# Audio-WestlakeU/FN-SSL

Measured on AMD Instinct MI355X. Metric: TF-frames/sec DP-IPD forward, 4-mic 257-bin x 300-frame, higher is better.
Workload: dtype f32; 1 GPU; BASELINE configs[1]: FN-SSL (online) DP-IPD forward, waveform->STFT->features->3x(full-band BiLSTM + narrow-band LSTM)->head; 32 utterances/GPU x 4 mics ('MM' = 6 pairs) x 257 bins x 300 frames, fp32; frame = one STFT frame of one utterance; stream_chunk_frames=0, utterances_per_gpu=32, global_batch=32, mics=4, pairs_per_utterance=6, frames=300, bins=257, parallelism=dp1 (utterance shards, no collective), chunk_pairs=0

## Files before the change

fn-ssl_amd/csrc/forward.hip:

```cpp
#include <algorithm>

#include "common.h"

namespace {

size_t align_up(size_t v, size_t a) { return (v + a - 1) / a * a; }

struct Plan {
  int chunk;
  size_t act_floats;
  size_t lstm_ws;
  size_t head_floats;
  size_t total;
};

Plan make_plan(int nb, int nf, int nt, int is_online, int chunk_pairs) {
  Plan p;
  p.chunk = (chunk_pairs <= 0 || chunk_pairs > nb) ? nb : chunk_pairs;
  p.act_floats = (size_t)p.chunk * nt * nf * 256;
  const size_t ws_full = fnssl_lstm_workspace_bytes_ex(p.chunk * nt, 128, 2, FNSSL_PRECISION_FP32);
  const size_t ws_narr = is_online ? fnssl_lstm_workspace_bytes_ex(p.chunk * nf, 256, 1, FNSSL_PRECISION_FP32)
                                   : fnssl_lstm_workspace_bytes_ex(p.chunk * nf, 128, 2, FNSSL_PRECISION_FP32);
  p.lstm_ws = align_up(std::max(ws_full, ws_narr), 256);
  p.head_floats = (size_t)p.chunk * (nt / FNSSL_SEG_FRAMES) * 2 * nf;
  p.total = 6 * align_up(p.act_floats * 4, 256) + p.lstm_ws + align_up(p.head_floats * 4, 256) + 256;
  return p;
}

}

extern "C" {

size_t fnssl_forward_workspace_bytes(int nb, int nf, int nt, int is_online, int chunk_pairs) {
  if (nb <= 0 || nf <= 0 || nt <= 0) return 0;
  return make_plan(nb, nf, nt, is_online, chunk_pairs).total;
}

int fnssl_forward(const fnssl_net* net, const float* x0, int nb, int nf, int nt, float* out, void* workspace,
                  size_t workspace_bytes, int chunk_pairs, void* stream) {
  FNSSL_REQUIRE(net && x0, "forward: null pointer");
  FNSSL_REQUIRE(nb > 0 && nf > 0 && nt > 0, "forward: empty problem (nb %d, nf %d, nt %d)", nb, nf, nt);
  if (nt / FNSSL_SEG_FRAMES == 0) return FNSSL_OK;
  FNSSL_REQUIRE(out, "forward: null output pointer");
  FNSSL_REQUIRE(net->input_size > 0 && net->input_size % 4 == 0, "forward: input_size %d must be a multiple of 4",
                net->input_size);
  FNSSL_REQUIRE(!net->doa_wt || nf == 256, "forward: the DOA layer needs nf = 256 (Linear(512, 180))");
  const Plan pl = make_plan(nb, nf, nt, net->is_online, chunk_pairs);
  if (!workspace || workspace_bytes < pl.total) {
    fnssl::set_error("forward: workspace %zu < %zu bytes", workspace_bytes, pl.total);
    return FNSSL_E_WORKSPACE;
  }
  char* wsb = static_cast<char*>(workspace);
  wsb = reinterpret_cast<char*>(align_up(reinterpret_cast<uintptr_t>(wsb), 256));
  const size_t act_bytes = align_up(pl.act_floats * 4, 256);
  float* F[2] = {reinterpret_cast<float*>(wsb), reinterpret_cast<float*>(wsb + act_bytes)};
  float* N[2] = {reinterpret_cast<float*>(wsb + 2 * act_bytes), reinterpret_cast<float*>(wsb + 3 * act_bytes)};
  float* Sf = reinterpret_cast<float*>(wsb + 4 * act_bytes);
  float* Sn = reinterpret_cast<float*>(wsb + 5 * act_bytes);
  float* lws = reinterpret_cast<float*>(wsb + 6 * act_bytes);
  float* head_tmp = reinterpret_cast<float*>(wsb + 6 * act_bytes + pl.lstm_ws);

  const int cin = net->input_size;
  const int nt2 = nt / FNSSL_SEG_FRAMES;
  const int narr_h = net->is_online ? 256 : 128;
  const int narr_dirs = net->is_online ? 1 : 2;
  const long long C = 256;
  const long long PS = (long long)nt * nf * C;
  const fnssl_view fl_by_full = {nullptr, PS, (long long)nf * C, C};
  const fnssl_view fl_by_narr = {nullptr, PS, C, (long long)nf * C};
  const fnssl_view nl_by_full = {nullptr, PS, C, (long long)nt * C};
  const fnssl_view nl_by_narr = {nullptr, PS, (long long)nt * C, C};
  auto with = [](fnssl_view v, const float* p) {
    v.p = p;
    return v;
  };

  for (int p0 = 0; p0 < nb; p0 += pl.chunk) {
    const int G = std::min(pl.chunk, nb - p0);
    const float* xc = x0 + (size_t)p0 * nt * nf * cin;
    for (int blk = 0; blk < 3; ++blk) {
      float* Fo = F[blk & 1];
      float* No = N[blk & 1];
      const float* Np = N[(blk + 1) & 1];
      fnssl_lstm_desc d = {};
      d.hidden = 128;
      d.ndir = 2;
      d.nseq = G * nt;
      d.q_inner = nt;
      d.nsteps = nf;
      if (blk == 0) {
        d.src0 = fnssl_view{xc, (long long)nt * nf * cin, (long long)nf * cin, cin};
        d.c0 = cin;
      } else {
        d.src0 = with(nl_by_full, Sn);
        d.c0 = 256;
      }
      d.out = Fo;
      d.out_so = fl_by_full.so;
      d.out_si = fl_by_full.si;
      d.out_st = fl_by_full.st;
      if (blk > 0) {
        d.skip = with(nl_by_full, Np);
        d.out_sum = Sf;
      }
      d.wpack[0] = net->wpack[blk][0][0];
      d.wpack[1] = net->wpack[blk][0][1];
      d.workspace = lws;
      d.workspace_bytes = pl.lstm_ws;
      d.fallback_count = net->fallback_count;
      d.tuning = net->tuning;
      int rc = fnssl_lstm_forward(&d, stream);
      if (rc != FNSSL_OK) return rc;
      fnssl_lstm_desc e = {};
      e.hidden = narr_h;
      e.ndir = narr_dirs;
      e.nseq = G * nf;
      e.q_inner = nf;
      e.nsteps = nt;
      e.c0 = 256;
      if (blk == 0) {
        e.src0 = with(fl_by_narr, Fo);
        e.src2 = fnssl_view{xc, (long long)nt * nf * cin, cin, (long long)nf * cin};
        e.c2 = cin;
      } else {
        e.src0 = with(fl_by_narr, Sf);
      }
      e.out = No;
      e.out_so = nl_by_narr.so;
      e.out_si = nl_by_narr.si;
      e.out_st = nl_by_narr.st;
      if (blk < 2) {
        e.skip = with(fl_by_narr, Fo);
        e.out_sum = Sn;
      }
      e.wpack[0] = net->wpack[blk][1][0];
      e.wpack[1] = net->wpack[blk][1][1];
      e.workspace = lws;
      e.workspace_bytes = pl.lstm_ws;
      e.fallback_count = net->fallback_count;
      e.tuning = net->tuning;
      rc = fnssl_lstm_forward(&e, stream);
      if (rc != FNSSL_OK) return rc;
    }
    if (nt2 > 0) {
      if (net->doa_wt) {
        int rc = fnssl_head(N[0], G, nf, nt, net->emb_w, net->emb_b, head_tmp, stream);
        if (rc != FNSSL_OK) return rc;
        rc = fnssl_linear(head_tmp, G * nt2, 2 * nf, net->doa_wt, net->doa_b, 180,
                          out + (size_t)p0 * nt2 * 180, stream);
        if (rc != FNSSL_OK) return rc;
      } else {
        int rc = fnssl_head(N[0], G, nf, nt, net->emb_w, net->emb_b, out + (size_t)p0 * nt2 * 2 * nf, stream);
        if (rc != FNSSL_OK) return rc;
      }
    }
  }
  return FNSSL_OK;
}

}
```

fn-ssl_amd/csrc/lstm.hip:

```cpp
#include <algorithm>
#include <cstdlib>
#include <cstring>
#include <vector>

#include "common.h"
#include "tuning.h"

#include "lstm_static.h"
#include "lstm_bf16.h"
#include "lstm_bf16w.h"
#include "lstm_split_static.h"

using namespace fnssl_lstm;

namespace fnssl_lstm {
extern template int launch_h<16>(int, const LstmParams&, int, int, hipStream_t);
extern template int launch_h<32>(int, const LstmParams&, int, int, hipStream_t);
extern template int launch_h<64>(int, const LstmParams&, int, int, hipStream_t);
extern template int launch_h<128>(int, const LstmParams&, int, int, hipStream_t);
extern template int launch_h<256>(int, const LstmParams&, int, int, hipStream_t);
extern template int launch_split_h<128>(int, const LstmParams&, int, int, hipStream_t);
extern template int launch_split_h<256>(int, const LstmParams&, int, int, hipStream_t);
int forward_save(LstmParams p, int H, int mode, hipStream_t st);
int forward_bf16(LstmParams p, int H, hipStream_t st);
// ... 308 lines not shown
                  "lstm_forward: the bf16 path takes one summed and one concatenated input of 16-channel blocks, "
                  "no fused residual / reserve / carry");
    p.quads_per_slice = bf16_quads_per_slice(d->c0, d->c2, H);
    p.chq = 0;
    p.pad = 0;
    report(FNSSL_LSTM_FAMILY_BF16);
    return forward_bf16(p, H, st);
  }
  if (d->precision == FNSSL_PRECISION_BF16W) {
    FNSSL_REQUIRE(!(mode & (kHas1 | kSum)) && !d->reserve && !d->carry_state && d->c0 % 16 == 0 && d->c2 % 16 == 0,
                  "lstm_forward: the wide bf16 path takes 16-channel input blocks, no fused residual / reserve / carry");
    auto mult8 = [](long long v) { return (v & 7) == 0; };
    const int fm = d->f32_mask & 7;
    FNSSL_REQUIRE(((fm & 1) || !d->c0 || (mult8(d->src0.so) && mult8(d->src0.si) && mult8(d->src0.st))) &&
                      ((fm & 2) || !d->c2 || (mult8(d->src2.so) && mult8(d->src2.si) && mult8(d->src2.st))) &&
                      ((fm & 4) || (mult8(d->out_so) && mult8(d->out_si) && mult8(d->out_st))),
                  "lstm_forward: strides of bf16 tensors must be multiples of 8 elements");
    return forward_bf16w(p, H, fm, ws.cluster.bytes, st, family);
  }
  FNSSL_REQUIRE(d->precision == FNSSL_PRECISION_FP32, "lstm_forward: unknown precision %d", d->precision);
  if (d->reserve) {
    FNSSL_REQUIRE((H == 128 || H == 256) && !(mode & (kHas1 | kSum)),
                  "lstm_forward: the reserve-saving forward needs hidden 128/256 and no src1 / out_sum");
    FNSSL_REQUIRE(d->reserve_bytes >= fnssl_lstm_reserve_bytes(d->nseq, H, d->ndir, d->nsteps) &&
                      (reinterpret_cast<uintptr_t>(d->reserve) & 15) == 0 &&
                      (long double)d->nsteps * (H / 16) * kReserveRecs * 1024 < 4.0e9L,
                  "lstm_forward: reserve buffer too small or misaligned");
    p.chq = 0;
    p.pad = 0;
    p.task0 = 0;
    p.task1 = tasks;
    p.wgs_per_dir = 0;
    if (d->variant == 0 && f32c_handles(p, H, mode)) {
      const int rc = forward_f32c(p, H, mode, ws.cluster.bytes, st);
      if (rc == FNSSL_OK) {
        report(FNSSL_LSTM_FAMILY_F32_CLUSTER);
        if (dry) return FNSSL_OK;
        guarded = true;
        p.guard = reinterpret_cast<const unsigned*>(p.cluster_ws);
      } else if (rc != kNoCluster) {
        return rc;
      }
    }
    report(FNSSL_LSTM_FAMILY_TRAIN);
    return dry ? FNSSL_OK : forward_save(p, H, mode, st);
  }

  if (d->variant == 0 && !(mode & kHas1) && f32c_handles(p, H, mode)) {
    const size_t cell_bytes = ws.cell.bytes;
    char* backup = reinterpret_cast<char*>(d->workspace) + ws.carry.off;
    const bool snap = p.carry && !dry;
    if (snap) FNSSL_HIP(hipMemcpyAsync(backup, p.cscratch, cell_bytes, hipMemcpyDeviceToDevice, st));
    const int rc = forward_f32c(p, H, mode, ws.cluster.bytes, st);
    if (rc == FNSSL_OK) {
      report(FNSSL_LSTM_FAMILY_F32_CLUSTER);
      if (rounds) *rounds = 1;
      if (dry) return FNSSL_OK;
      guarded = true;
      p.guard = reinterpret_cast<const unsigned*>(p.cluster_ws);
      if (snap) {
        const long long n4 = (long long)(cell_bytes / 16);
        hipLaunchKernelGGL(restore_cell_kernel, dim3((unsigned)std::min<long long>((n4 + 255) / 256, 2048)), dim3(256), 0, st, p.guard,
                           reinterpret_cast<const float4*>(backup), reinterpret_cast<float4*>(p.cscratch), n4);
        FNSSL_CHECK_LAUNCH("restore_cell_kernel");
      }
    } else if (rc != kNoCluster) {
      return rc;
    }
  }

  auto launch_range = [&](int variant, int t0, int t1) -> int {
    const Variant& vr = kVariants[variant];
    p.task0 = t0;
    p.task1 = t1;
    p.wgs_per_dir = (t1 - t0 + vr.NW - 1) / vr.NW;
    const int nwg = p.wgs_per_dir * d->ndir;
    ++nlaunch;
    if (d->variant == 0 && !fnssl::tune(FNSSL_TUNE_LSTM_NO_STATIC)) {
      int rc = kNoStatic;
      if (H == 128) rc = launch_static_h128(p, mode, vr.NW, nwg, st);
      if (H == 256) {
        const bool s3 = !p.ablate && !fnssl::tune(FNSSL_TUNE_NO_STATIC3) && (mode == kSum || mode == 0 || mode == (kHas2 | kSum)) &&
                        ((d->c2 == 0 && !(mode & kHas2)) || (d->c2 == 4 && (mode & kHas2)));
        if (vr.NW == 12 && d->c0 == 256 && !p.carry && s3) {
          LstmParams p2 = p;
          const long long n4 = (long long)(H / 16) * p.quads_per_slice * 4 * 64;
          char* dst = reinterpret_cast<char*>(d->workspace) + ws.stream.off;
          FNSSL_REQUIRE((size_t)d->ndir * n4 * 16 <= ws.stream.bytes, "lstm_forward: no room for the interleaved weight stream");
          const bool s4 = !fnssl::tune(FNSSL_TUNE_NO_STATIC4);
          for (int di = 0; di < d->ndir; ++di) {
            float4* o = reinterpret_cast<float4*>(dst + (size_t)di * n4 * 16);
            if (!dry) {
              if (s4)
                hipLaunchKernelGGL(quad_stream_kernel, dim3((unsigned)((n4 + 255) / 256)), dim3(256), 0, st,
                                   reinterpret_cast<const float4*>(p.wpack[di]), p.quads_per_slice, n4, o);
              else
                hipLaunchKernelGGL(pair_stream_kernel, dim3((unsigned)((n4 + 255) / 256)), dim3(256), 0, st,
                                   reinterpret_cast<const float4*>(p.wpack[di]), p.quads_per_slice, n4, o);
            }
            p2.wpack[di] = reinterpret_cast<const float*>(o);
          }
          FNSSL_CHECK_LAUNCH("pair_stream_kernel");
          rc = s4 ? launch_static4_h256(p2, mode, nwg, st) : launch_static3_h256(p2, mode, nwg, st);
          if (rc != kNoStatic) {
            report(s4 ? FNSSL_LSTM_FAMILY_STATIC4 : FNSSL_LSTM_FAMILY_STATIC3);
            return rc;
          }
        }
        rc = launch_static_h256(p, mode, vr.NW, nwg, st);
      }
      if (rc == kNoStatic && !fnssl::tune(FNSSL_TUNE_NO_STATIC_IPDNET)) rc = launch_static_ipdnet(p, mode, H, vr.NW, nwg, st);
      if (rc != kNoStatic) {
        report(FNSSL_LSTM_FAMILY_STATIC);
        return rc;
      }
    }
    report(FNSSL_LSTM_FAMILY_GENERIC);
    p.chq = 0;
    p.pad = 0;
    if (vr.ring) choose_chunk(p.quads_per_slice, vr, p.chq, p.pad);
    switch (H) {
      case 16: return launch_h<16>(variant, p, mode, nwg, st);
      case 32: return launch_h<32>(variant, p, mode, nwg, st);
      case 64: return launch_h<64>(variant, p, mode, nwg, st);
      case 128: return launch_h<128>(variant, p, mode, nwg, st);
      default: return launch_h<256>(variant, p, mode, nwg, st);
    }
  };

  if (d->variant != 0 || H < 128) {
    const int variant = d->variant ? d->variant : default_variant(H);
    FNSSL_REQUIRE(variant >= 1 && variant <= kNumVariants, "lstm_forward: unknown variant %d", variant);
    const int rc = launch_range(variant, 0, tasks);
    if (rounds && !guarded) *rounds = nlaunch;
    return rc;
  }
  if (const int forced = default_variant_override(H)) {
    const int rc = launch_range(forced, 0, tasks);
    if (rounds && !guarded) *rounds = nlaunch;
    return rc;
  }

  const int ncu = fnssl::device_cus();
  auto launch_split = [&](int split, int t0, int t1, bool static_only) -> int {
    const int nw = split == 4 ? 8 : 4, groups_per_wg = nw / split;
    p.task0 = t0;
    p.task1 = t1;
    p.wgs_per_dir = (t1 - t0 + groups_per_wg - 1) / groups_per_wg;
    const Variant vr{nw, split == 4 ? 8 : 4, 1};
    choose_chunk(p.quads_per_slice, vr, p.chq, p.pad, split);
    const int nwg = p.wgs_per_dir * d->ndir;
    if (rounds) *rounds = 1;
    if (!p.carry && !(mode & kHas1)) {
      const int rc = launch_split_static(p, H, nw, split, mode, 0, nwg, st);
      if (rc != kNoStatic) report(FNSSL_LSTM_FAMILY_SPLIT_STATIC);
      if (rc != kNoStatic || static_only) return rc;
    } else if (static_only) {
      return kNoStatic;
    }
    report(FNSSL_LSTM_FAMILY_SPLIT);
    return H == 128 ? launch_split_h<128>(split, p, mode, nwg, st) : launch_split_h<256>(split, p, mode, nwg, st);
  };
  {
    const long long total = (long long)tasks * d->ndir;
    if (const int f = fnssl::tune(FNSSL_TUNE_LSTM_SPLIT, 1, 4)) {
      if (f != 1) return launch_split(f == 3 ? 2 : f, 0, tasks, false);
    } else {
// ... 44 lines not shown
```

fn-ssl_amd/csrc/lstm_static4.h:

```cpp
#pragma once

#include "lstm_static.h"

#pragma clang fp contract(off)

namespace fnssl_lstm {

constexpr int static4_blocks_in_chunk(int qe, int chq, int nv0, int ns2, int ns) {
  int n = 0;
  for (int q = qe - chq + 1; q <= qe; ++q) {
    const bool x = q >= 1 && q <= nv0;
    const bool h = q >= 1 + nv0 + ns2 && q < 1 + nv0 + ns2 + ns;
    n += (x || h) ? 1 : 0;
  }
  return n;
}

template <int H, int NW, int NV0, int NS2, int CHQ, int PAD, int MODE, int XD = 4, bool PF4 = false>
__global__ void __launch_bounds__(NW * 64) lstm_static4_kernel(const LstmParams p) {
  FNSSL_GUARDED_KERNEL(p);
  constexpr int NS = H / 16, NP = NS / 4;
  constexpr int NB = NV0 + NS;
  constexpr bool HAS2 = (MODE & kHas2) != 0, SUM = (MODE & kSum) != 0;
  static_assert(!(MODE & kHas1) && HAS2 == (NS2 > 0) && NS % 4 == 0 && NS2 <= 1, "modes");
  constexpr int QPS = 1 + NV0 + NS2 + NS;
  constexpr int VQ = QPS + PAD;
  static_assert(VQ % CHQ == 0, "chunks must tile the (padded) slice quad");
  constexpr int CH = 16 * CHQ;
  constexpr int M = (CH + NW - 1) / NW;
  static_assert(NB % XD == 0 && XD <= NV0, "the operand ring depth must divide the block count");
  static_assert(PAD < CHQ, "a chunk of padding only would have no operand load to count the DMA by");
  extern __shared__ __attribute__((aligned(16))) char smem[];

  const int lane = threadIdx.x & 63;
  const int n = lane & 15, g = lane >> 4;
  const int w = __builtin_amdgcn_readfirstlane((int)(threadIdx.x >> 6));
  const int dir = blockIdx.x / p.wgs_per_dir;
  const int wg = blockIdx.x - dir * p.wgs_per_dir;
  const int task = p.task0 + wg * NW + w;
  int q = task * 16 + n;
  const bool valid = q < p.nseq && task < p.task1;
  if (q >= p.nseq) q = p.nseq - 1;
  const long long qo = q / p.q_inner, qi = q - qo * p.q_inner;

  unsigned vo0 = 0, vo2 = 0, voo = 0, vok = 0, voo2 = 0;
  const rsrc_t rx0 = split_addr(p.src0.p, qo * p.src0.so + qi * p.src0.si, 4 * g, vo0);
  const rsrc_t rx2 = HAS2 ? split_addr(p.src2.p, qo * p.src2.so + qi * p.src2.si, g, vo2) : rx0;
  const rsrc_t rsk = SUM ? split_addr(p.skip.p, qo * p.skip.so + qi * p.skip.si, dir * H + 4 * g, vok) : rx0;
  const rsrc_t ro = split_addr(p.out, qo * p.out_so + qi * p.out_si, dir * H + 4 * g, voo);
  const rsrc_t ro2 = SUM ? split_addr(p.out_sum, qo * p.out_so + qi * p.out_si, dir * H + 4 * g, voo2) : ro;
  const rsrc_t rzero = __builtin_amdgcn_make_buffer_rsrc(const_cast<float*>(p.out), 0, 0, 0x00020000);
  const rsrc_t rc = make_rsrc(cell_record<NS>(p.cscratch, p.ntasks, dir, task < p.task1 ? task : p.ntasks + w));
  const rsrc_t rw = make_rsrc(p.wpack[dir]);
  const unsigned st0 = (unsigned)(p.src0.st * 4), st2 = HAS2 ? (unsigned)(p.src2.st * 4) : 0u;
  const unsigned sto = (unsigned)(p.out_st * 4), stk = SUM ? (unsigned)(p.skip.st * 4) : 0u;
  const unsigned vlane = lane * 16;
  const bool rev = dir == 1;

  const unsigned lds0 = (unsigned)(uintptr_t)smem;
  char* const lds_rd = smem + lane * 16;
  int dslot = 0, rslot = 0;
  int src_rec = 0;
  int src_vq = 0;
  auto issue_dma = [&]() {
#pragma unroll
    for (int m = 0; m < M; ++m) {
      const int r = w + m * NW;
      if (r < CH && src_vq * 16 + r < QPS * 16) {
        const unsigned soff = (unsigned)(src_rec + r) * 1024u;
        const unsigned ld = lds0 + (unsigned)(dslot * CH + r) * 1024u;
        asm volatile("s_mov_b32 m0, %2\n\ts_nop 0\n\tbuffer_load_dwordx4 %0, %1, %3 offen lds" ::"v"(vlane), "s"(rw),
                     "s"(__builtin_amdgcn_readfirstlane(ld)), "s"(__builtin_amdgcn_readfirstlane(soff))
                     : "memory");
      }
    }
    dslot ^= 1;
    src_vq += CHQ;
    src_rec += CH;
    if (src_vq == VQ) {
      src_vq = 0;
      src_rec -= PAD * 16;
      if (src_rec == NP * QPS * 16) src_rec = 0;
    }
  };
  issue_dma();
  asm volatile("s_waitcnt vmcnt(0)\n\ts_barrier" ::: "memory");
  issue_dma();
  const char* cb = lds_rd;
  auto rec = [&](auto ql, int j) { return *reinterpret_cast<const v4f*>(cb + decltype(ql)::value * 16384 + j * 1024); };
  v4f a0 = rec(ic<0>{}, 0), a1 = rec(ic<0>{}, 1);

  const v4f zero4 = v4f{0.f, 0.f, 0.f, 0.f};
  v4f acc[4][4];

  auto ring_step = [&](auto qi_c) {
    constexpr int QL = decltype(qi_c)::value % CHQ;
    if constexpr (QL + 1 < CHQ) {
      a0 = rec(ic<QL + 1>{}, 0);
      a1 = rec(ic<QL + 1>{}, 1);
    }
  };
  auto ring_end = [&](auto qi_c) {
    constexpr int QI = decltype(qi_c)::value, QL = QI % CHQ;
    if constexpr (QL + 1 == CHQ) {
      constexpr int K = static4_blocks_in_chunk(QI, CHQ, NV0, NS2, NS);
#ifdef FNSSL_BUILD_ABLATE
      asm volatile("s_waitcnt vmcnt(0)" ::: "memory");
#else
      if constexpr (K >= 3)
        asm volatile("s_waitcnt vmcnt(3)" ::: "memory");
      else if constexpr (K == 2)
        asm volatile("s_waitcnt vmcnt(2)" ::: "memory");
      else if constexpr (K == 1)
        asm volatile("s_waitcnt vmcnt(1)" ::: "memory");
      else
        asm volatile("s_waitcnt vmcnt(0)" ::: "memory");
#endif
      asm volatile("s_waitcnt lgkmcnt(0)\n\ts_barrier" ::: "memory");
      issue_dma();
      rslot ^= 1;
      cb = lds_rd + rslot * (CH * 1024);
      a0 = rec(ic<0>{}, 0);
      a1 = rec(ic<0>{}, 1);
    }
  };
#define SQUAD4(QI, B0, B1, B2, B3)                                                \
  do {                                                                            \
    const v4f a2_ = rec(ic<(QI) % CHQ>{}, 2), a3_ = rec(ic<(QI) % CHQ>{}, 3);     \
    __builtin_amdgcn_sched_barrier(0);                                            \
    MFMA4(acc[0], a0, B0);                                                        \
    MFMA4(acc[0], a1, B1);                                                        \
    const v4f b0_ = rec(ic<(QI) % CHQ>{}, 4), b1_ = rec(ic<(QI) % CHQ>{}, 5);     \
    __builtin_amdgcn_sched_barrier(0);                                            \
    MFMA4(acc[0], a2_, B2);                                                       \
    MFMA4(acc[0], a3_, B3);                                                       \
    const v4f b2_ = rec(ic<(QI) % CHQ>{}, 6), b3_ = rec(ic<(QI) % CHQ>{}, 7);     \
    __builtin_amdgcn_sched_barrier(0);                                            \
    MFMA4(acc[1], b0_, B0);                                                       \
    MFMA4(acc[1], b1_, B1);                                                       \
    const v4f c0_ = rec(ic<(QI) % CHQ>{}, 8), c1_ = rec(ic<(QI) % CHQ>{}, 9);     \
    __builtin_amdgcn_sched_barrier(0);                                            \
    MFMA4(acc[1], b2_, B2);                                                       \
    MFMA4(acc[1], b3_, B3);                                                       \
    const v4f c2_ = rec(ic<(QI) % CHQ>{}, 10), c3_ = rec(ic<(QI) % CHQ>{}, 11);   \
    __builtin_amdgcn_sched_barrier(0);                                            \
    MFMA4(acc[2], c0_, B0);                                                       \
    MFMA4(acc[2], c1_, B1);                                                       \
    const v4f d0_ = rec(ic<(QI) % CHQ>{}, 12), d1_ = rec(ic<(QI) % CHQ>{}, 13);   \
    __builtin_amdgcn_sched_barrier(0);                                            \
    MFMA4(acc[2], c2_, B2);                                                       \
    MFMA4(acc[2], c3_, B3);                                                       \
    const v4f d2_ = rec(ic<(QI) % CHQ>{}, 14), d3_ = rec(ic<(QI) % CHQ>{}, 15);   \
    __builtin_amdgcn_sched_barrier(0);                                            \
    MFMA4(acc[3], d0_, B0);                                                       \
    MFMA4(acc[3], d1_, B1);                                                       \
    ring_step(ic<(QI)>{});                                                        \
    __builtin_amdgcn_sched_barrier(0);                                            \
    MFMA4(acc[3], d2_, B2);                                                       \
    MFMA4(acc[3], d3_, B3);                                                       \
    ring_end(ic<(QI)>{});                                                         \
  } while (0)
#define SQUAD4_1(QI, B0)                                                                          \
  do {                                                                                            \
    const v4f b0_ = rec(ic<(QI) % CHQ>{}, 4), c0_ = rec(ic<(QI) % CHQ>{}, 8), d0_ = rec(ic<(QI) % CHQ>{}, 12); \
    MFMA4(acc[0], a0, B0);                                                                        \
    MFMA4(acc[1], b0_, B0);                                                                       \
    MFMA4(acc[2], c0_, B0);                                                                       \
    MFMA4(acc[3], d0_, B0);                                                                       \
    ring_step(ic<(QI)>{});                                                                        \
    ring_end(ic<(QI)>{});                                                                         \
  } while (0)

  v4f br[XD];
  {
    const unsigned tt0 = rev ? p.nsteps - 1 : 0;
    static_for<XD>([&](auto v) { br[v.value] = bld4(rx0, vo0, tt0 * st0 + 64 * v.value); });
  }

  for (int step = 0; step < p.nsteps; ++step) {
    const unsigned tt = rev ? p.nsteps - 1 - step : step;
    const unsigned ttn = step + 1 < p.nsteps ? (rev ? tt - 1 : tt + 1) : tt;
    const unsigned o0 = tt * st0, o2 = tt * st2, oo = tt * sto, ok = tt * stk;
    const unsigned op = (rev ? tt + 1 : tt - 1) * sto;
    const rsrc_t rh = step > 0 ? ro : rzero;
    float xs2 = 0.f;
    if (NS2) xs2 = bld1(rx2, vo2, o2);

    for (int pr = 0; pr < NP; ++pr) {
      const int s0 = 4 * pr;
#ifdef FNSSL_BUILD_ABLATE
      const bool skip_ring = (p.ablate & 2) != 0;
#else
      constexpr bool skip_ring = false;
#endif
      v4f cprev = zero4, skipv = zero4;
      v4f cpf[PF4 ? 4 : 1], skf[PF4 ? 4 : 1];
      if constexpr (PF4) static_for<4>([&](auto s_) { cpf[s_.value] = zero4; skf[s_.value] = zero4; });
      const bool last = pr + 1 == NP;
      const unsigned nx = (last ? ttn : tt) * st0;
      acc[0][0] = a0;
      acc[0][1] = a1;
      static_for<14>([&](auto j) {
        constexpr int J = decltype(j)::value + 2;
        acc[J / 4][J % 4] = rec(ic<0>{}, J);
      });
      ring_step(ic<0>{});
      ring_end(ic<0>{});
      static_for<NB>([&](auto bc) {
        constexpr int B = decltype(bc)::value;
        constexpr int QI = B < NV0 ? 1 + B : 1 + NS2 + B;
        if constexpr (NS2 > 0 && B == NV0) SQUAD4_1(1 + NV0, xs2);
        const v4f ob = br[B % XD];
        constexpr int BN = (B + XD) % NB;
        if (!skip_ring) {
          if constexpr (B + XD < NB) {
            if constexpr (BN < NV0)
              br[B % XD] = bld4(rx0, vo0, o0 + 64 * BN);
            else
              br[B % XD] = bld4(rh, voo, op + 64 * (BN - NV0));
          } else {
            static_assert(BN < NV0, "the wrapped requests are input blocks");
            br[B % XD] = bld4(rx0, vo0, nx + 64 * BN);
          }
        }
        if constexpr (!PF4 && B == NB - 4) {
          if (step > 0) cprev = bld4(rc, vlane, s0 * 1024);
          if (SUM) skipv = bld4(rsk, vok, ok + 64 * s0);
        }
        if constexpr (PF4 && B == NB - 3) {
          static_for<4>([&](auto s_) {
            constexpr int S = decltype(s_)::value;
            if (step > 0) cpf[S] = bld4(rc, vlane, (s0 + S) * 1024);
            if (SUM) skf[S] = bld4(rsk, vok, ok + 64 * (s0 + S));
          });
        }
        SQUAD4(QI, ob.x, ob.y, ob.z, ob.w);
      });
      static_for<PAD>([&](auto u) {
        ring_step(ic<QPS + decltype(u)::value>{});
        ring_end(ic<QPS + decltype(u)::value>{});
      });
      static_for<4>([&](auto sc) {
        constexpr int S = decltype(sc)::value;
        const v4f ig = sigmoid4(acc[S][0]), fg = sigmoid4(acc[S][1]), gg = tanh4(acc[S][2]), og = sigmoid4(acc[S][3]);
        v4f cp_cur = cprev, sk_cur = skipv;
        if constexpr (PF4) {
          cp_cur = cpf[S];
          sk_cur = skf[S];
        } else if constexpr (S < 3) {
          if (step > 0) cprev = bld4(rc, vlane, (s0 + S + 1) * 1024);
          if (SUM) skipv = bld4(rsk, vok, ok + 64 * (s0 + S + 1));
        }
        const v4f cn = cell4(fg, cp_cur, ig, gg);
        v4f hn = mul_rn4(og, tanh4(cn));
        asm("" : "+v"(hn.x), "+v"(hn.y), "+v"(hn.z), "+v"(hn.w));
        bst4(cn, rc, vlane, (s0 + S) * 1024);
        if (valid) {
          bst4(hn, ro, voo, oo + 64 * (s0 + S));
          if (SUM) bst4(add_rn4(hn, sk_cur), ro2, voo2, oo + 64 * (s0 + S));
        }
      });
    }
  }
  asm volatile("s_waitcnt vmcnt(0)" ::: "memory");
#undef SQUAD4
#undef SQUAD4_1
}

template <int H, int NW, int NV0, int NS2, int CHQ, int PAD, int MODE, int XD = 4, bool PF4 = false>
int launch_static4_k(const LstmParams& p, int nwg, hipStream_t st) {
  if (p.dry) return FNSSL_OK;
  const size_t lds = (size_t)2 * CHQ * 16384;
  static_assert(2 * CHQ * 16384 <= 160 * 1024, "ring does not fit the LDS");
  auto k = lstm_static4_kernel<H, NW, NV0, NS2, CHQ, PAD, MODE, XD, PF4>;
  if (lds > 48 * 1024)
    FNSSL_HIP(hipFuncSetAttribute(reinterpret_cast<const void*>(k), hipFuncAttributeMaxDynamicSharedMemorySize, (int)lds));
  hipLaunchKernelGGL(k, dim3(nwg), dim3(NW * 64), lds, st, p);
  FNSSL_CHECK_LAUNCH("lstm_static4_kernel");
  return FNSSL_OK;
}

}
```

fn-ssl_amd/csrc/lstm_static4_h256.hip:

```cpp
#include "lstm_static4.h"

namespace fnssl_lstm {

int launch_static4_h256(const LstmParams& p_in, int mode, int nwg, hipStream_t st) {
  LstmParams p = p_in;
#ifdef FNSSL_BUILD_ABLATE
  p.ablate = env_int("FNSSL_STATIC3_ABL", 1, 3);
#endif
  if (p.c0 == 256 && p.c2 == 0 && mode == kSum) return launch_static4_k<256, 12, 16, 0, 3, 0, kSum, 4, true>(p, nwg, st);
  if (p.c0 == 256 && p.c2 == 0 && mode == 0) return launch_static4_k<256, 12, 16, 0, 3, 0, 0, 4, true>(p, nwg, st);
  if (p.c0 == 256 && p.c2 == 4 && mode == (kHas2 | kSum))
    return launch_static4_k<256, 12, 16, 1, 3, 2, kHas2 | kSum>(p, nwg, st);
  return kNoStatic;
}

}
```

fn-ssl_amd/csrc/runtime.hip:

```cpp
#include <atomic>
#include <cstring>
#include <map>
#include <mutex>
#include <string>
#include <vector>

#include "common.h"
#include "tuning.h"

namespace fnssl {

int device_cus() {
  static std::mutex mu;
  static int cache[64] = {0};
  int dev = 0;
  if (hipGetDevice(&dev) != hipSuccess || dev < 0 || dev >= 64) return 256;
  std::lock_guard<std::mutex> lk(mu);
  if (cache[dev] == 0) {
    int n = 0;
    if (hipDeviceGetAttribute(&n, hipDeviceAttributeMultiprocessorCount, dev) != hipSuccess || n <= 0) n = 256;
    cache[dev] = n;
  }
  return cache[dev];
}


static thread_local char g_err[512] = "";

namespace {
std::mutex g_tuning_mu;
fnssl_tuning g_default_tuning = {sizeof(fnssl_tuning), {0}};
std::atomic<unsigned> g_tuning_version{1};
thread_local fnssl_tuning g_thread_tuning = {sizeof(fnssl_tuning), {0}};
thread_local unsigned g_thread_version = 0;
thread_local const fnssl_tuning* g_call_tuning = nullptr;
const char* const kTuneNames[] = {
    "LSTM_NO_STATIC",
    "NO_STATIC3",
    "NO_STATIC2",
    "NO_STATIC_IPDNET",
    "LSTM_SPLIT",
    "SPLIT4_MAX_H256",
    "LSTM_VARIANT_H128",
    "LSTM_VARIANT_H256",
    "LSTM_CHQ",
    "NO_F32_CLUSTER",
    "NO_F32C_B1",
    "TRAIN_NO_F32_CLUSTER",
    "F32C_NO_ROTATE",
    "F32C_PRIO",
    "NO_CLUSTER",
    "NO_CLUSTER_B1",
    "NO_CLUSTER_H128",
    "CLUSTER_SPREAD",
    "BF16P_DRAIN",
    "BF16W_SOLO",
    "BWD_NO_CLUSTER",
    "BWD_CLUSTER_MIN_GROUPS",
    "BWD_CLUSTER_NO_ROTATE",
    "BWDC_NO_PREFETCH",
    "BWDC_NO_TOKEN",
    "BWDC_WAVES16",
    "FWD_RING",
    "BWD_RING",
    "TRAIN_SPLIT",
    "TRAIN_NO_STATIC",
    "NO_FWD2",
    "NO_BWD2",
    "SN_SCALAR",
    "STFT_PER_FRAME",
    "CLUSTER_SPIN_LIMIT",
    "CLUSTER_TEST_STALL",
    "RESERVED_CUS",
    "NO_F32_SMALL",
    "F32C_MIN_GROUPS",
    "F32C_GATE_SPLIT",
    "CLUSTER_FULL_TILES",
    "NO_STATIC4"};
constexpr int kTuneNamed = (int)(sizeof(kTuneNames) / sizeof(kTuneNames[0]));
static_assert(kTuneNamed <= FNSSL_TUNE_COUNT, "more knob names than slots");
static_assert(kTuneNamed == FNSSL_TUNE_NO_STATIC4 + 1, "knob names out of step with include/fnssl.h");
}

const fnssl_tuning& tuning() {
  if (g_call_tuning) return *g_call_tuning;
  const unsigned v = g_tuning_version.load(std::memory_order_acquire);
  if (v != g_thread_version) {
    std::lock_guard<std::mutex> lk(g_tuning_mu);
    g_thread_tuning = g_default_tuning;
    g_thread_version = g_tuning_version.load(std::memory_order_relaxed);
  }
  return g_thread_tuning;
}

TuningScope::TuningScope(const fnssl_tuning* t) : prev_(g_call_tuning), active_(false) {
  if (t && t->struct_bytes == sizeof(fnssl_tuning)) {
    g_call_tuning = t;
    active_ = true;
  }
}
TuningScope::~TuningScope() {
  if (active_) g_call_tuning = prev_;
}

void set_error(const char* fmt, ...) {
  va_list ap;
  va_start(ap, fmt);
  vsnprintf(g_err, sizeof(g_err), fmt, ap);
  va_end(ap);
}

namespace {
struct Rec {
  const char* name;
  double flops;
  hipEvent_t e0, e1;
};
std::mutex g_mu;
std::vector<Rec> g_recs;
bool g_timing = false;
char g_select[64] = "";
}

TimedLaunch::TimedLaunch(const char* name, hipStream_t s, double flops)
    : name_(name), s_(s), flops_(flops) {
  if (!g_timing || !name) return;
  if (g_select[0] && std::strcmp(g_select, name) != 0) return;
  if (hipEventCreate(&e0_) != hipSuccess) {
    e0_ = nullptr;
    return;
  }
  (void)hipEventRecord(e0_, s_);
}

TimedLaunch::~TimedLaunch() {
  if (!e0_) return;
  hipEvent_t e1 = nullptr;
  if (hipEventCreate(&e1) != hipSuccess) {
    (void)hipEventDestroy(e0_);
    return;
  }
  (void)hipEventRecord(e1, s_);
  std::lock_guard<std::mutex> lk(g_mu);
  g_recs.push_back(Rec{name_, flops_, e0_, e1});
}

}

extern "C" int fnssl_tuning_set(const fnssl_tuning* t) {
  FNSSL_REQUIRE(!t || t->struct_bytes == sizeof(fnssl_tuning), "tuning_set: struct_bytes %u, this library's fnssl_tuning has %zu",
                t ? t->struct_bytes : 0u, sizeof(fnssl_tuning));
  std::lock_guard<std::mutex> lk(fnssl::g_tuning_mu);
  fnssl::g_default_tuning = t ? *t : fnssl_tuning{sizeof(fnssl_tuning), {0}};
  fnssl::g_tuning_version.fetch_add(1, std::memory_order_release);
  return FNSSL_OK;
}

extern "C" int fnssl_tuning_get(fnssl_tuning* t) {
  FNSSL_REQUIRE(t != nullptr, "tuning_get: NULL");
  std::lock_guard<std::mutex> lk(fnssl::g_tuning_mu);
  *t = fnssl::g_default_tuning;
  return FNSSL_OK;
}

// ... 141 lines not shown
```

include/fnssl.h:

```cpp
#ifndef FNSSL_H_
#define FNSSL_H_

#include <stddef.h>

#ifdef __cplusplus
extern "C" {
#endif

#define FNSSL_ABI_VERSION 19

#define FNSSL_OK 0
#define FNSSL_E_INVALID (-1)
#define FNSSL_E_HIP (-2)
#define FNSSL_E_WORKSPACE (-3)

#define FNSSL_CH_MODE_M 0
#define FNSSL_CH_MODE_MM 1

#define FNSSL_WIN_LEN 512
#define FNSSL_HOP 256
#define FNSSL_NBIN 257
#define FNSSL_NF 256
#define FNSSL_SEG_FRAMES 12

int fnssl_abi_version(void);
const char* fnssl_last_error(void);


#define FNSSL_TUNE_LSTM_NO_STATIC 0
#define FNSSL_TUNE_NO_STATIC3 1
#define FNSSL_TUNE_NO_STATIC2 2
#define FNSSL_TUNE_NO_STATIC_IPDNET 3
#define FNSSL_TUNE_LSTM_SPLIT 4
#define FNSSL_TUNE_SPLIT4_MAX_H256 5
#define FNSSL_TUNE_LSTM_VARIANT_H128 6
#define FNSSL_TUNE_LSTM_VARIANT_H256 7
#define FNSSL_TUNE_LSTM_CHQ 8
#define FNSSL_TUNE_NO_F32_CLUSTER 9
#define FNSSL_TUNE_NO_F32C_B1 10
#define FNSSL_TUNE_TRAIN_NO_F32_CLUSTER 11
#define FNSSL_TUNE_F32C_NO_ROTATE 12
#define FNSSL_TUNE_F32C_PRIO 13
#define FNSSL_TUNE_NO_CLUSTER 14
#define FNSSL_TUNE_NO_CLUSTER_B1 15
#define FNSSL_TUNE_NO_CLUSTER_H128 16
#define FNSSL_TUNE_CLUSTER_SPREAD 17
#define FNSSL_TUNE_BF16P_DRAIN 18
#define FNSSL_TUNE_BF16W_SOLO 19
#define FNSSL_TUNE_BWD_NO_CLUSTER 20
#define FNSSL_TUNE_BWD_CLUSTER_MIN_GROUPS 21
#define FNSSL_TUNE_BWD_CLUSTER_NO_ROTATE 22
#define FNSSL_TUNE_BWDC_NO_PREFETCH 23
#define FNSSL_TUNE_BWDC_NO_TOKEN 24
#define FNSSL_TUNE_BWDC_WAVES16 25
#define FNSSL_TUNE_FWD_RING 26
#define FNSSL_TUNE_BWD_RING 27
#define FNSSL_TUNE_TRAIN_SPLIT 28
#define FNSSL_TUNE_TRAIN_NO_STATIC 29
#define FNSSL_TUNE_NO_FWD2 30
#define FNSSL_TUNE_NO_BWD2 31
#define FNSSL_TUNE_SN_SCALAR 32
#define FNSSL_TUNE_STFT_PER_FRAME 33
#define FNSSL_TUNE_CLUSTER_SPIN_LIMIT 34
#define FNSSL_TUNE_CLUSTER_TEST_STALL 35
#define FNSSL_TUNE_RESERVED_CUS 36
#define FNSSL_TUNE_NO_F32_SMALL 37
#define FNSSL_TUNE_F32C_MIN_GROUPS 38
#define FNSSL_TUNE_F32C_GATE_SPLIT 39
#define FNSSL_TUNE_CLUSTER_FULL_TILES 40
#define FNSSL_TUNE_NO_STATIC4 41
#define FNSSL_TUNE_COUNT 48

typedef struct fnssl_tuning {
  unsigned struct_bytes;
  int knob[FNSSL_TUNE_COUNT];
} fnssl_tuning;

int fnssl_tuning_set(const fnssl_tuning* t);
int fnssl_tuning_get(fnssl_tuning* t);
const char* fnssl_tuning_name(int index);

int fnssl_occupy_cus(int nblocks, int lds_bytes, unsigned* stop, int max_ms, void* stream);


int fnssl_num_frames(int ns);

int fnssl_num_pairs(int nch, int ch_mode);

int fnssl_stft(const float* sig, int nb, int ns, int nch,
               long long sb, long long sn, long long sc,
               float* spec, float* magsum, void* stream);

int fnssl_num_frames_ex(int ns, int hop, int center);
int fnssl_stft_ex(const float* sig, int nb, int ns, int nch,
                  long long sb, long long sn, long long sc, int hop, int center,
                  float* spec, float* magsum, void* stream);

int fnssl_forgetting_coefs(int nt, int sample_length, float* a, float* b);

int fnssl_pair_features(const float* spec, const float* magsum,
                        const float* coef_a, const float* coef_b,
                        int nb, int nch, int nt, int ch_mode, float eps,
                        float* mu, float* x, int layout, void* stream);

int fnssl_nchw_to_seq(const float* x, int n, int c, int nf, int nt, float* y, void* stream);


typedef struct {
  const float* p;
  long long so, si, st;
} fnssl_view;

typedef struct {
  fnssl_view src0, src1, src2;
  int c0, c2;
  float* out;
  long long out_so, out_si, out_st;
  fnssl_view skip;
  float* out_sum;
  int hidden;
  int ndir;
  int nseq;
  int q_inner;
  int nsteps;
  const float* wpack[2];
  float* workspace;
  size_t workspace_bytes;
  int variant;
  float* reserve;
  size_t reserve_bytes;
  int carry_state;
  int precision;
  int f32_mask;
  unsigned* fallback_count;
  const fnssl_tuning* tuning;
} fnssl_lstm_desc;

#define FNSSL_PRECISION_FP32 0
#define FNSSL_PRECISION_BF16 1
#define FNSSL_PRECISION_BF16W 2

size_t fnssl_lstm_packed_floats_bf16w(int c0, int c2, int hidden);
int fnssl_lstm_pack_bf16w(const float* w_ih, const float* w_hh, const float* b_ih, const float* b_hh,
                          int c0, int c2, int hidden, float* packed);

size_t fnssl_lstm_packed_floats_bf16(int c0, int c2, int hidden);
int fnssl_lstm_pack_bf16(const float* w_ih, const float* w_hh, const float* b_ih, const float* b_hh,
                         int c0, int c2, int hidden, float* packed);

size_t fnssl_lstm_packed_floats(int c0, int c2, int hidden);

int fnssl_lstm_pack(const float* w_ih, const float* w_hh, const float* b_ih, const float* b_hh,
                    int c0, int c2, int hidden, float* packed);
// ... 356 lines not shown
```

Measured before the change: 17920 frames/s.

## Fuse full-band skip sum into narrow-band static4 LSTM input loads

For blocks 1 and 2 the full-band LSTM no longer writes a separate summed tensor Sf. When the planner picks the static4 family, the narrow-band LSTM instead reads both the full-band output and the previous narrow-band output and adds them while loading its input (new kHas1 mode). When its skip equals src0, the skip is derived from the same address and offset, so the loads are not issued twice. This removes one write and one read of a full activation tensor per block, at the cost of an extra input stream inside the recurrent kernel and deeper vmcnt accounting. A PRODUCER_SUM knob restores the old path.

```diff
diff --git a/fn-ssl_amd/csrc/forward.hip b/fn-ssl_amd/csrc/forward.hip
--- a/fn-ssl_amd/csrc/forward.hip
+++ b/fn-ssl_amd/csrc/forward.hip
@@ -1,6 +1,7 @@
 #include <algorithm>
 
 #include "common.h"
+#include "tuning.h"
 
 namespace {
 
@@ -75,6 +76,8 @@
     return v;
   };
 
+  fnssl::TuningScope tuning_of_this_call(net->tuning);
+  const bool producer_sum = fnssl::tune(FNSSL_TUNE_PRODUCER_SUM) != 0;
   for (int p0 = 0; p0 < nb; p0 += pl.chunk) {
     const int G = std::min(pl.chunk, nb - p0);
     const float* xc = x0 + (size_t)p0 * nt * nf * cin;
@@ -82,6 +85,42 @@
       float* Fo = F[blk & 1];
       float* No = N[blk & 1];
       const float* Np = N[(blk + 1) & 1];
+      fnssl_lstm_desc e = {};
+      e.hidden = narr_h;
+      e.ndir = narr_dirs;
+      e.nseq = G * nf;
+      e.q_inner = nf;
+      e.nsteps = nt;
+      e.c0 = 256;
+      e.out = No;
+      e.out_so = nl_by_narr.so;
+      e.out_si = nl_by_narr.si;
+      e.out_st = nl_by_narr.st;
+      if (blk < 2) {
+        e.skip = with(fl_by_narr, Fo);
+        e.out_sum = Sn;
+      }
+      e.wpack[0] = net->wpack[blk][1][0];
+      e.wpack[1] = net->wpack[blk][1][1];
+      e.workspace = lws;
+      e.workspace_bytes = pl.lstm_ws;
+      e.fallback_count = net->fallback_count;
+      e.tuning = net->tuning;
+      bool consumer_sum = false;
+      if (blk == 0) {
+        e.src0 = with(fl_by_narr, Fo);
+        e.src2 = fnssl_view{xc, (long long)nt * nf * cin, cin, (long long)nf * cin};
+        e.c2 = cin;
+      } else {
+        e.src0 = with(fl_by_narr, Fo);
+        e.src1 = with(nl_by_narr, Np);
+        int family = 0;
+        consumer_sum = !producer_sum && fnssl_lstm_plan(&e, &family, nullptr) == FNSSL_OK && family == FNSSL_LSTM_FAMILY_STATIC4;
+        if (!consumer_sum) {
+          e.src0 = with(fl_by_narr, Sf);
+          e.src1 = fnssl_view{};
+        }
+      }
       fnssl_lstm_desc d = {};
       d.hidden = 128;
       d.ndir = 2;
@@ -99,7 +138,7 @@
       d.out_so = fl_by_full.so;
       d.out_si = fl_by_full.si;
       d.out_st = fl_by_full.st;
-      if (blk > 0) {
+      if (blk > 0 && !consumer_sum) {
         d.skip = with(nl_by_full, Np);
         d.out_sum = Sf;
       }
@@ -111,34 +150,6 @@
       d.tuning = net->tuning;
       int rc = fnssl_lstm_forward(&d, stream);
       if (rc != FNSSL_OK) return rc;
-      fnssl_lstm_desc e = {};
-      e.hidden = narr_h;
-      e.ndir = narr_dirs;
-      e.nseq = G * nf;
-      e.q_inner = nf;
-      e.nsteps = nt;
-      e.c0 = 256;
-      if (blk == 0) {
-        e.src0 = with(fl_by_narr, Fo);
-        e.src2 = fnssl_view{xc, (long long)nt * nf * cin, cin, (long long)nf * cin};
-        e.c2 = cin;
-      } else {
-        e.src0 = with(fl_by_narr, Sf);
-      }
-      e.out = No;
-      e.out_so = nl_by_narr.so;
-      e.out_si = nl_by_narr.si;
-      e.out_st = nl_by_narr.st;
-      if (blk < 2) {
-        e.skip = with(fl_by_narr, Fo);
-        e.out_sum = Sn;
-      }
-      e.wpack[0] = net->wpack[blk][1][0];
-      e.wpack[1] = net->wpack[blk][1][1];
-      e.workspace = lws;
-      e.workspace_bytes = pl.lstm_ws;
-      e.fallback_count = net->fallback_count;
-      e.tuning = net->tuning;
       rc = fnssl_lstm_forward(&e, stream);
       if (rc != FNSSL_OK) return rc;
     }
diff --git a/fn-ssl_amd/csrc/lstm.hip b/fn-ssl_amd/csrc/lstm.hip
--- a/fn-ssl_amd/csrc/lstm.hip
+++ b/fn-ssl_amd/csrc/lstm.hip
@@ -414,7 +414,10 @@
       if (H == 256) {
         const bool s3 = !p.ablate && !fnssl::tune(FNSSL_TUNE_NO_STATIC3) && (mode == kSum || mode == 0 || mode == (kHas2 | kSum)) &&
                         ((d->c2 == 0 && !(mode & kHas2)) || (d->c2 == 4 && (mode & kHas2)));
-        if (vr.NW == 12 && d->c0 == 256 && !p.carry && s3) {
+        const bool same_skip = d->skip.p == d->src0.p && d->skip.so == d->src0.so && d->skip.si == d->src0.si && d->skip.st == d->src0.st;
+        const bool s4two = !p.ablate && !fnssl::tune(FNSSL_TUNE_NO_STATIC3) && !fnssl::tune(FNSSL_TUNE_NO_STATIC4) && d->c2 == 0 &&
+                           (mode == kHas1 || (mode == (kHas1 | kSum) && same_skip));
+        if (vr.NW == 12 && d->c0 == 256 && !p.carry && (s3 || s4two)) {
           LstmParams p2 = p;
           const long long n4 = (long long)(H / 16) * p.quads_per_slice * 4 * 64;
           char* dst = reinterpret_cast<char*>(d->workspace) + ws.stream.off;
diff --git a/fn-ssl_amd/csrc/lstm_static4.h b/fn-ssl_amd/csrc/lstm_static4.h
--- a/fn-ssl_amd/csrc/lstm_static4.h
+++ b/fn-ssl_amd/csrc/lstm_static4.h
@@ -6,12 +6,14 @@
 
 namespace fnssl_lstm {
 
-constexpr int static4_blocks_in_chunk(int qe, int chq, int nv0, int ns2, int ns) {
+constexpr int static4_blocks_in_chunk(int qe, int chq, int nv0, int ns2, int ns, int xd = 4, bool has1 = false) {
   int n = 0;
   for (int q = qe - chq + 1; q <= qe; ++q) {
     const bool x = q >= 1 && q <= nv0;
     const bool h = q >= 1 + nv0 + ns2 && q < 1 + nv0 + ns2 + ns;
-    n += (x || h) ? 1 : 0;
+    if (!(x || h)) continue;
+    const int b = x ? q - 1 : nv0 + q - (1 + nv0 + ns2);
+    n += (has1 && (b + xd) % (nv0 + ns) < nv0) ? 2 : 1;
   }
   return n;
 }
@@ -22,7 +24,10 @@
   constexpr int NS = H / 16, NP = NS / 4;
   constexpr int NB = NV0 + NS;
   constexpr bool HAS2 = (MODE & kHas2) != 0, SUM = (MODE & kSum) != 0;
-  static_assert(!(MODE & kHas1) && HAS2 == (NS2 > 0) && NS % 4 == 0 && NS2 <= 1, "modes");
+  constexpr bool HAS1 = (MODE & kHas1) != 0;
+  constexpr bool SK0 = HAS1 && SUM;
+  constexpr bool PFSK = PF4 && !SK0;
+  static_assert(!(HAS1 && HAS2) && HAS2 == (NS2 > 0) && NS % 4 == 0 && NS2 <= 1, "modes");
   constexpr int QPS = 1 + NV0 + NS2 + NS;
   constexpr int VQ = QPS + PAD;
   static_assert(VQ % CHQ == 0, "chunks must tile the (padded) slice quad");
@@ -43,17 +48,20 @@
   if (q >= p.nseq) q = p.nseq - 1;
   const long long qo = q / p.q_inner, qi = q - qo * p.q_inner;
 
-  unsigned vo0 = 0, vo2 = 0, voo = 0, vok = 0, voo2 = 0;
+  unsigned vo0 = 0, vo1 = 0, vo2 = 0, voo = 0, vok = 0, voo2 = 0;
   const rsrc_t rx0 = split_addr(p.src0.p, qo * p.src0.so + qi * p.src0.si, 4 * g, vo0);
+  const rsrc_t rx1 = HAS1 ? split_addr(p.src1.p, qo * p.src1.so + qi * p.src1.si, 4 * g, vo1) : rx0;
   const rsrc_t rx2 = HAS2 ? split_addr(p.src2.p, qo * p.src2.so + qi * p.src2.si, g, vo2) : rx0;
-  const rsrc_t rsk = SUM ? split_addr(p.skip.p, qo * p.skip.so + qi * p.skip.si, dir * H + 4 * g, vok) : rx0;
+  const rsrc_t rsk = (SUM && !SK0) ? split_addr(p.skip.p, qo * p.skip.so + qi * p.skip.si, dir * H + 4 * g, vok) : rx0;
+  if (SK0) vok = vo0 + (unsigned)(dir * H * 4);
   const rsrc_t ro = split_addr(p.out, qo * p.out_so + qi * p.out_si, dir * H + 4 * g, voo);
   const rsrc_t ro2 = SUM ? split_addr(p.out_sum, qo * p.out_so + qi * p.out_si, dir * H + 4 * g, voo2) : ro;
   const rsrc_t rzero = __builtin_amdgcn_make_buffer_rsrc(const_cast<float*>(p.out), 0, 0, 0x00020000);
   const rsrc_t rc = make_rsrc(cell_record<NS>(p.cscratch, p.ntasks, dir, task < p.task1 ? task : p.ntasks + w));
   const rsrc_t rw = make_rsrc(p.wpack[dir]);
   const unsigned st0 = (unsigned)(p.src0.st * 4), st2 = HAS2 ? (unsigned)(p.src2.st * 4) : 0u;
-  const unsigned sto = (unsigned)(p.out_st * 4), stk = SUM ? (unsigned)(p.skip.st * 4) : 0u;
+  const unsigned st1 = HAS1 ? (unsigned)(p.src1.st * 4) : 0u;
+  const unsigned sto = (unsigned)(p.out_st * 4), stk = SK0 ? st0 : SUM ? (unsigned)(p.skip.st * 4) : 0u;
   const unsigned vlane = lane * 16;
   const bool rev = dir == 1;
 
@@ -69,9 +77,12 @@
       if (r < CH && src_vq * 16 + r < QPS * 16) {
         const unsigned soff = (unsigned)(src_rec + r) * 1024u;
         const unsigned ld = lds0 + (unsigned)(dslot * CH + r) * 1024u;
+#pragma clang diagnostic push
+#pragma clang diagnostic ignored "-Winline-asm"
         asm volatile("s_mov_b32 m0, %2\n\ts_nop 0\n\tbuffer_load_dwordx4 %0, %1, %3 offen lds" ::"v"(vlane), "s"(rw),
                      "s"(__builtin_amdgcn_readfirstlane(ld)), "s"(__builtin_amdgcn_readfirstlane(soff))
-                     : "memory");
+                     : "memory", "m0");
+#pragma clang diagnostic pop
       }
     }
     dslot ^= 1;
@@ -103,11 +114,18 @@
   auto ring_end = [&](auto qi_c) {
     constexpr int QI = decltype(qi_c)::value, QL = QI % CHQ;
     if constexpr (QL + 1 == CHQ) {
-      constexpr int K = static4_blocks_in_chunk(QI, CHQ, NV0, NS2, NS);
+      constexpr int K = static4_blocks_in_chunk(QI, CHQ, NV0, NS2, NS, XD, HAS1);
 #ifdef FNSSL_BUILD_ABLATE
       asm volatile("s_waitcnt vmcnt(0)" ::: "memory");
 #else
-      if constexpr (K >= 3)
+      static_assert(K <= 2 * CHQ && (HAS1 || K <= 3), "loads counted behind one chunk's DMA request");
+      if constexpr (K >= 6)
+        asm volatile("s_waitcnt vmcnt(6)" ::: "memory");
+      else if constexpr (K == 5)
+        asm volatile("s_waitcnt vmcnt(5)" ::: "memory");
+      else if constexpr (K == 4)
+        asm volatile("s_waitcnt vmcnt(4)" ::: "memory");
+      else if constexpr (K == 3)
         asm volatile("s_waitcnt vmcnt(3)" ::: "memory");
       else if constexpr (K == 2)
         asm volatile("s_waitcnt vmcnt(2)" ::: "memory");
@@ -171,16 +189,19 @@
     ring_end(ic<(QI)>{});                                                                         \
   } while (0)
 
-  v4f br[XD];
+  v4f br[XD], bs[HAS1 ? XD : 1];
   {
     const unsigned tt0 = rev ? p.nsteps - 1 : 0;
-    static_for<XD>([&](auto v) { br[v.value] = bld4(rx0, vo0, tt0 * st0 + 64 * v.value); });
+    static_for<XD>([&](auto v) {
+      br[v.value] = bld4(rx0, vo0, tt0 * st0 + 64 * v.value);
+      if constexpr (HAS1) bs[v.value] = bld4(rx1, vo1, tt0 * st1 + 64 * v.value);
+    });
   }
 
   for (int step = 0; step < p.nsteps; ++step) {
     const unsigned tt = rev ? p.nsteps - 1 - step : step;
     const unsigned ttn = step + 1 < p.nsteps ? (rev ? tt - 1 : tt + 1) : tt;
-    const unsigned o0 = tt * st0, o2 = tt * st2, oo = tt * sto, ok = tt * stk;
+    const unsigned o0 = tt * st0, o1 = tt * st1, o2 = tt * st2, oo = tt * sto, ok = tt * stk;
     const unsigned op = (rev ? tt + 1 : tt - 1) * sto;
     const rsrc_t rh = step > 0 ? ro : rzero;
     float xs2 = 0.f;
@@ -194,10 +215,11 @@
       constexpr bool skip_ring = false;
 #endif
       v4f cprev = zero4, skipv = zero4;
-      v4f cpf[PF4 ? 4 : 1], skf[PF4 ? 4 : 1];
-      if constexpr (PF4) static_for<4>([&](auto s_) { cpf[s_.value] = zero4; skf[s_.value] = zero4; });
+      v4f cpf[PF4 ? 4 : 1], skf[PFSK ? 4 : 1];
+      if constexpr (PF4) static_for<4>([&](auto s_) { cpf[s_.value] = zero4; });
+      if constexpr (PFSK) static_for<4>([&](auto s_) { skf[s_.value] = zero4; });
       const bool last = pr + 1 == NP;
-      const unsigned nx = (last ? ttn : tt) * st0;
+      const unsigned nx = (last ? ttn : tt) * st0, nx1 = (last ? ttn : tt) * st1;
       acc[0][0] = a0;
       acc[0][1] = a1;
       static_for<14>([&](auto j) {
@@ -210,28 +232,35 @@
         constexpr int B = decltype(bc)::value;
         constexpr int QI = B < NV0 ? 1 + B : 1 + NS2 + B;
         if constexpr (NS2 > 0 && B == NV0) SQUAD4_1(1 + NV0, xs2);
-        const v4f ob = br[B % XD];
+        v4f ob = br[B % XD];
+        if constexpr (HAS1 && B < NV0) ob = add_rn4(ob, bs[B % XD]);
         constexpr int BN = (B + XD) % NB;
         if (!skip_ring) {
           if constexpr (B + XD < NB) {
-            if constexpr (BN < NV0)
+            if constexpr (BN < NV0) {
               br[B % XD] = bld4(rx0, vo0, o0 + 64 * BN);
-            else
+              if constexpr (HAS1) bs[B % XD] = bld4(rx1, vo1, o1 + 64 * BN);
+            } else {
               br[B % XD] = bld4(rh, voo, op + 64 * (BN - NV0));
+            }
           } else {
             static_assert(BN < NV0, "the wrapped requests are input blocks");
             br[B % XD] = bld4(rx0, vo0, nx + 64 * BN);
+            if constexpr (HAS1) bs[B % XD] = bld4(rx1, vo1, nx1 + 64 * BN);
           }
         }
-        if constexpr (!PF4 && B == NB - 4) {
-          if (step > 0) cprev = bld4(rc, vlane, s0 * 1024);
-          if (SUM) skipv = bld4(rsk, vok, ok + 64 * s0);
+        if constexpr (B == NB - 4) {
+          if constexpr (!PF4)
+            if (step > 0) cprev = bld4(rc, vlane, s0 * 1024);
+          if constexpr (!PFSK)
+            if (SUM) skipv = bld4(rsk, vok, ok + 64 * s0);
         }
         if constexpr (PF4 && B == NB - 3) {
           static_for<4>([&](auto s_) {
             constexpr int S = decltype(s_)::value;
             if (step > 0) cpf[S] = bld4(rc, vlane, (s0 + S) * 1024);
-            if (SUM) skf[S] = bld4(rsk, vok, ok + 64 * (s0 + S));
+            if constexpr (PFSK)
+              if (SUM) skf[S] = bld4(rsk, vok, ok + 64 * (s0 + S));
           });
         }
         SQUAD4(QI, ob.x, ob.y, ob.z, ob.w);
@@ -244,12 +273,13 @@
         constexpr int S = decltype(sc)::value;
         const v4f ig = sigmoid4(acc[S][0]), fg = sigmoid4(acc[S][1]), gg = tanh4(acc[S][2]), og = sigmoid4(acc[S][3]);
         v4f cp_cur = cprev, sk_cur = skipv;
-        if constexpr (PF4) {
-          cp_cur = cpf[S];
-          sk_cur = skf[S];
-        } else if constexpr (S < 3) {
-          if (step > 0) cprev = bld4(rc, vlane, (s0 + S + 1) * 1024);
-          if (SUM) skipv = bld4(rsk, vok, ok + 64 * (s0 + S + 1));
+        if constexpr (PF4) cp_cur = cpf[S];
+        if constexpr (PFSK) sk_cur = skf[S];
+        if constexpr (S < 3) {
+          if constexpr (!PF4)
+            if (step > 0) cprev = bld4(rc, vlane, (s0 + S + 1) * 1024);
+          if constexpr (!PFSK)
+            if (SUM) skipv = bld4(rsk, vok, ok + 64 * (s0 + S + 1));
         }
         const v4f cn = cell4(fg, cp_cur, ig, gg);
         v4f hn = mul_rn4(og, tanh4(cn));
diff --git a/fn-ssl_amd/csrc/lstm_static4_h256.hip b/fn-ssl_amd/csrc/lstm_static4_h256.hip
--- a/fn-ssl_amd/csrc/lstm_static4_h256.hip
+++ b/fn-ssl_amd/csrc/lstm_static4_h256.hip
@@ -9,6 +9,10 @@
 #endif
   if (p.c0 == 256 && p.c2 == 0 && mode == kSum) return launch_static4_k<256, 12, 16, 0, 3, 0, kSum, 4, true>(p, nwg, st);
   if (p.c0 == 256 && p.c2 == 0 && mode == 0) return launch_static4_k<256, 12, 16, 0, 3, 0, 0, 4, true>(p, nwg, st);
+  if (p.c0 == 256 && p.c2 == 0 && mode == kHas1) return launch_static4_k<256, 12, 16, 0, 3, 0, kHas1, 4, true>(p, nwg, st);
+  if (p.c0 == 256 && p.c2 == 0 && mode == (kHas1 | kSum) && p.skip.p == p.src0.p && p.skip.so == p.src0.so &&
+      p.skip.si == p.src0.si && p.skip.st == p.src0.st)
+    return launch_static4_k<256, 12, 16, 0, 3, 0, kHas1 | kSum, 4, true>(p, nwg, st);
   if (p.c0 == 256 && p.c2 == 4 && mode == (kHas2 | kSum))
     return launch_static4_k<256, 12, 16, 1, 3, 2, kHas2 | kSum>(p, nwg, st);
   return kNoStatic;
diff --git a/fn-ssl_amd/csrc/runtime.hip b/fn-ssl_amd/csrc/runtime.hip
--- a/fn-ssl_amd/csrc/runtime.hip
+++ b/fn-ssl_amd/csrc/runtime.hip
@@ -76,10 +76,11 @@
     "F32C_MIN_GROUPS",
     "F32C_GATE_SPLIT",
     "CLUSTER_FULL_TILES",
-    "NO_STATIC4"};
+    "NO_STATIC4",
+    "PRODUCER_SUM"};
 constexpr int kTuneNamed = (int)(sizeof(kTuneNames) / sizeof(kTuneNames[0]));
 static_assert(kTuneNamed <= FNSSL_TUNE_COUNT, "more knob names than slots");
-static_assert(kTuneNamed == FNSSL_TUNE_NO_STATIC4 + 1, "knob names out of step with include/fnssl.h");
+static_assert(kTuneNamed == FNSSL_TUNE_PRODUCER_SUM + 1, "knob names out of step with include/fnssl.h");
 }
 
 const fnssl_tuning& tuning() {
diff --git a/include/fnssl.h b/include/fnssl.h
--- a/include/fnssl.h
+++ b/include/fnssl.h
@@ -69,6 +69,7 @@
 #define FNSSL_TUNE_F32C_GATE_SPLIT 39
 #define FNSSL_TUNE_CLUSTER_FULL_TILES 40
 #define FNSSL_TUNE_NO_STATIC4 41
+#define FNSSL_TUNE_PRODUCER_SUM 42
 #define FNSSL_TUNE_COUNT 48
 
 typedef struct fnssl_tuning {
```

Result: no change. 18000 frames/s (median of 6 runs) (+0.5%).
